# palonso/MAEST

Measured on AMD Instinct MI355X. Metric: clips/sec (10s@16kHz, 96-mel) MAEST-10s fwd+bwd, higher is better.
Workload: dtype bf16; 1 GPU; maest_10s_random_weights_pretrain training step (BASELINE configs[2]): mixup + fwd + BCE + bwd + AdamW; arch=passt_s_swa_p16_128_ap476 (DeiT-B distilled, 85.9M params), random init, per_gpu_batch=256, global_batch=256, s_patchout_t=30, classes=400, hip_graph_forward=False, parallelism=dp1

## Files before the change

maest_amd/csrc/embed.hip:

```cpp
#include "common.h"

namespace maest {

constexpr int PE_D = 768;
constexpr int PE_K = 16;
constexpr int PE_S = 10;

__device__ __forceinline__ uint32_t stripe_bits(const int32_t* __restrict__ t_stripes, int n_t,
                                                const int32_t* __restrict__ f_stripes, int n_f, int b, int frow,
                                                int tcol) {
    for (int k = 0; k < n_f; ++k) {
        int st = f_stripes[((int64_t)b * n_f + k) * 2];
        const int w = f_stripes[((int64_t)b * n_f + k) * 2 + 1];
        st = st < 0 ? 0 : st;
        if (frow >= st && frow < st + w) return 0xffffu;
    }
    uint32_t bits = 0;
    for (int k = 0; k < n_t; ++k) {
        int st = t_stripes[((int64_t)b * n_t + k) * 2];
        const int w = t_stripes[((int64_t)b * n_t + k) * 2 + 1];
        st = st < 0 ? 0 : st;
        int lo = st - tcol, hi = st + w - tcol;
        lo = lo < 0 ? 0 : lo;
        hi = hi > 16 ? 16 : hi;
// ... 77 lines not shown
    const int c = threadIdx.x * 4;
    const int b0 = blockIdx.y * TA_BCHUNK;
    const int b1 = b0 + TA_BCHUNK < B ? b0 + TA_BCHUNK : B;
    if (n < 2) {
        const float* tok = n == 0 ? cls_token : dist_token;
        float4 o;
        o.x = tok[c] + new_pos[n * PE_D + c];
        o.y = tok[c + 1] + new_pos[n * PE_D + c + 1];
        o.z = tok[c + 2] + new_pos[n * PE_D + c + 2];
        o.w = tok[c + 3] + new_pos[n * PE_D + c + 3];
        for (int b = b0; b < b1; ++b) *reinterpret_cast<float4*>(x0 + ((int64_t)b * Ntok + n) * PE_D + c) = o;
        return;
    }
    const int j = n - 2;
    const int f = tok_ft[2 * j];
    const int tcol = toffset + tok_ft[2 * j + 1];
    float tp[4], fp[4];
#pragma unroll
    for (int e = 0; e < 4; ++e) {
        tp[e] = time_pos[(int64_t)(c + e) * Tt + tcol];
        fp[e] = freq_pos[(int64_t)(c + e) * Fg + f];
    }
    for (int b = b0; b < b1; ++b) {
        const float4 p = *reinterpret_cast<const float4*>(patches + ((int64_t)b * P + j) * PE_D + c);
        float4 o;
        o.x = (p.x + tp[0]) + fp[0];
        o.y = (p.y + tp[1]) + fp[1];
        o.z = (p.z + tp[2]) + fp[2];
        o.w = (p.w + tp[3]) + fp[3];
        *reinterpret_cast<float4*>(x0 + ((int64_t)b * Ntok + n) * PE_D + c) = o;
    }
}

constexpr int TAB_SLICES = 2;
template <bool TABLES>
__global__ __launch_bounds__(192) void token_assemble_bwd_kernel(const float* __restrict__ dx0, int B, int Fg, int P,
                                                                 int Tt, int toffset,
                                                                 const int32_t* __restrict__ tok_ft,
                                                                 void* __restrict__ dpatches, int dtype,
                                                                 float* __restrict__ d_cls, float* __restrict__ d_dist,
                                                                 float* __restrict__ d_new_pos,
                                                                 float* __restrict__ d_freq_pos,
                                                                 float* __restrict__ d_time_pos) {
    const int Ntok = 2 + P;
    const int n = TABLES ? blockIdx.x : blockIdx.x + 2;
    const int c = threadIdx.x * 4;
    const int per = (B + (int)gridDim.y - 1) / (int)gridDim.y;
    const int b0 = blockIdx.y * per;
    const int b1 = b0 + per < B ? b0 + per : B;
    float s[4] = {0.0f, 0.0f, 0.0f, 0.0f};
    const bool store = n >= 2 && dpatches != nullptr;
    auto one = [&](int b, const float4& g) {
        s[0] += g.x; s[1] += g.y; s[2] += g.z; s[3] += g.w;
        if (store) {
            const int64_t o = ((int64_t)b * P + (n - 2)) * PE_D + c;
            if (dtype == MAEST_BF16) {
                chunk8 v;
                v[0] = pack_bf2(g.x, g.y); v[1] = pack_bf2(g.z, g.w);
                *reinterpret_cast<chunk8*>(reinterpret_cast<bf16_t*>(dpatches) + o) = v;
            } else {
                *reinterpret_cast<float4*>(reinterpret_cast<float*>(dpatches) + o) = g;
            }
        }
    };
    const int64_t bstride = (int64_t)Ntok * PE_D;
    const float* src = dx0 + (int64_t)n * PE_D + c;
    int b = b0;
    for (; b + 4 <= b1; b += 4) {
        float4 g[4];
#pragma unroll
        for (int u = 0; u < 4; ++u) g[u] = *reinterpret_cast<const float4*>(src + (b + u) * bstride);
#pragma unroll
        for (int u = 0; u < 4; ++u) one(b + u, g[u]);
    }
    for (; b < b1; ++b) one(b, *reinterpret_cast<const float4*>(src + b * bstride));
    if (!TABLES || b0 >= b1) return;
    if (n == 0) {
#pragma unroll
        for (int e = 0; e < 4; ++e) { unsafeAtomicAdd(d_cls + c + e, s[e]); unsafeAtomicAdd(d_new_pos + c + e, s[e]); }
    } else if (n == 1) {
#pragma unroll
        for (int e = 0; e < 4; ++e) { unsafeAtomicAdd(d_dist + c + e, s[e]); unsafeAtomicAdd(d_new_pos + PE_D + c + e, s[e]); }
    } else {
        const int j = n - 2;
        const int f = tok_ft[2 * j];
        const int tcol = toffset + tok_ft[2 * j + 1];
#pragma unroll
        for (int e = 0; e < 4; ++e) {
            unsafeAtomicAdd(d_freq_pos + (int64_t)(c + e) * Fg + f, s[e]);
            unsafeAtomicAdd(d_time_pos + (int64_t)(c + e) * Tt + tcol, s[e]);
        }
    }
}

__global__ __launch_bounds__(64) void token_tables_ordered_kernel(const float* __restrict__ dx0, int B, int Fg, int P, int Tt, int toffset,
                                                                  const int32_t* __restrict__ tok_ft, float* __restrict__ d_cls,
                                                                  float* __restrict__ d_dist, float* __restrict__ d_new_pos,
                                                                  float* __restrict__ d_freq_pos, float* __restrict__ d_time_pos) {
    const int Ntok = 2 + P;
    const int d = blockIdx.x;
    const int c = blockIdx.y * 256 + threadIdx.x * 4;
    const int64_t bstride = (int64_t)Ntok * PE_D;
    float s[4] = {0.0f, 0.0f, 0.0f, 0.0f};
    auto token = [&](int n) {
        const float* src = dx0 + (int64_t)n * PE_D + c;
        int b = 0;
        for (; b + 16 <= B; b += 16) {
            float4 g[16];
#pragma unroll
// ... 235 lines not shown
    int32_t* mlist = lam ? moff + B + 1 : nullptr;
    hipLaunchKernelGGL(col2im_prep_kernel, dim3(1), dim3(256), 0, (hipStream_t)stream, tok_ft, P, Fp, Tp, perm, B, lut, moff,
                       mlist);
    const dim3 grid((unsigned)(((int64_t)F * T + 255) / 256), (unsigned)B);
#define MAEST_COL2IM(GT, XT)                                                                                               \
    hipLaunchKernelGGL((col2im_kernel<GT, XT>), grid, dim3(256), 0, (hipStream_t)stream, (const GT*)dcols, B, F, T,       \
                       stride_f, stride_t, Fp, Tp, P, lam, lut, moff, mlist, t_stripes, n_t, f_stripes, n_f, (XT*)dx)
    if (dtype == MAEST_BF16 && dx_dtype == MAEST_F16) MAEST_COL2IM(bf16_t, _Float16);
    else if (dtype == MAEST_BF16) MAEST_COL2IM(bf16_t, float);
    else if (dx_dtype == MAEST_F16) MAEST_COL2IM(float, _Float16);
    else MAEST_COL2IM(float, float);
#undef MAEST_COL2IM
    return check_launch("maest_patch_im2col_bwd");
}

extern "C" int maest_token_assemble(const float* patches, const float* cls_token, const float* dist_token,
                                    const float* new_pos, const float* freq_pos, const float* time_pos, int Fg, int Tt,
                                    int toffset, const int32_t* tok_ft, int B, int P, float* x0, void* stream) {
    MAEST_REQUIRE(patches && cls_token && dist_token && new_pos && freq_pos && time_pos && x0 && tok_ft,
                  "maest_token_assemble: null pointer");
    MAEST_REQUIRE(B > 0 && P > 0 && Fg > 0 && Tt > 0 && toffset >= 0, "maest_token_assemble: bad shape");
    hipLaunchKernelGGL(token_assemble_kernel, dim3(2 + P, (B + TA_BCHUNK - 1) / TA_BCHUNK), dim3(PE_D / 4), 0,
                       (hipStream_t)stream, patches, cls_token, dist_token, new_pos, freq_pos, time_pos, Tt, toffset,
                       tok_ft, B, Fg, P, x0);
    return check_launch("maest_token_assemble");
}

extern "C" int maest_token_assemble_bwd(const float* dx0, int B, int P, int Fg, int Tt, int toffset,
                                        const int32_t* tok_ft, void* dpatches, int dtype, float* d_cls, float* d_dist,
                                        float* d_new_pos, float* d_freq_pos, float* d_time_pos, void* stream) {
    MAEST_REQUIRE(dx0 && d_cls && d_dist && d_new_pos && d_freq_pos && d_time_pos && tok_ft,
                  "maest_token_assemble_bwd: null pointer");
    MAEST_REQUIRE(B > 0 && P > 0 && Fg > 0 && Tt > 0, "maest_token_assemble_bwd: bad shape");
    static_assert(PE_D == 192 * 4, "token_assemble_bwd_kernel: one thread per four channels");
    if (option(MAEST_OPT_DETERMINISTIC) != 0) {
        if (dpatches != nullptr)
            hipLaunchKernelGGL(token_assemble_bwd_kernel<false>, dim3(P, TAB_SLICES), dim3(192), 0, (hipStream_t)stream, dx0, B, Fg, P, Tt,
                               toffset, tok_ft, dpatches, dtype, d_cls, d_dist, d_new_pos, d_freq_pos, d_time_pos);
        static_assert(PE_D == 3 * 256, "token_tables_ordered_kernel: three channel groups of 64 lanes x 4");
        hipLaunchKernelGGL(token_tables_ordered_kernel, dim3(2 + Fg + Tt, 3), dim3(64), 0, (hipStream_t)stream, dx0, B, Fg, P, Tt, toffset,
                           tok_ft, d_cls, d_dist, d_new_pos, d_freq_pos, d_time_pos);
        return check_launch("maest_token_assemble_bwd(ordered)");
    }
    hipLaunchKernelGGL(token_assemble_bwd_kernel<true>, dim3(2 + P, TAB_SLICES), dim3(192), 0, (hipStream_t)stream,
                       dx0, B, Fg, P, Tt, toffset, tok_ft, dpatches, dtype, d_cls, d_dist, d_new_pos, d_freq_pos,
                       d_time_pos);
    return check_launch("maest_token_assemble_bwd");
}

extern "C" int maest_spec_mask(float* x, int B, int F, int T, const int32_t* t_stripes, int n_t,
                               const int32_t* f_stripes, int n_f, void* stream) {
    MAEST_REQUIRE(x, "maest_spec_mask: null pointer");
    MAEST_REQUIRE(n_t >= 0 && n_f >= 0 && (n_t == 0 || t_stripes) && (n_f == 0 || f_stripes),
                  "maest_spec_mask: bad stripe lists");
    if (n_t + n_f == 0) return MAEST_OK;
    hipLaunchKernelGGL(spec_mask_kernel, dim3(B, n_t + n_f), dim3(256), 0, (hipStream_t)stream, x, F, T, t_stripes,
                       n_t, f_stripes, n_f);
    return check_launch("maest_spec_mask");
}

extern "C" int maest_melfile_assemble(const uint16_t* frames, const int64_t* row_start, const int32_t* frames_read,
                                      int B, int n_bands, int T, int normalize, float norm_mean, float norm_div,
                                      float* out, void* stream) {
    MAEST_REQUIRE(frames && row_start && frames_read && out, "maest_melfile_assemble: null pointer");
    MAEST_REQUIRE(B > 0 && T > 0 && n_bands > 0 && n_bands <= 96, "maest_melfile_assemble: bad shape B=%d T=%d bands=%d",
                  B, T, n_bands);
    hipLaunchKernelGGL(melfile_assemble_kernel, dim3((T + 63) / 64, B), dim3(256), 64 * 97 * 4, (hipStream_t)stream, frames,
                       row_start, frames_read, n_bands, T, normalize, norm_mean, norm_div, out);
    return check_launch("maest_melfile_assemble");
}
```

maest_amd/csrc/gemm.hip:

```cpp
#include "common.h"
#include "gemm256_epi.h"

namespace maest {

constexpr int GEMM_BM = 128;
constexpr int GEMM_BN = 128;
constexpr int GEMM_ROWB = 128;
constexpr int GEMM_PITCH = 144;
constexpr int GEMM_TILE_BYTES = GEMM_BM * GEMM_PITCH;
constexpr int GEMM_SMEM_BYTES = 4 * GEMM_TILE_BYTES;

struct GemmParams {
    const char* A;
    const char* B;
    void* C;
    const float* bias;
    const void* aux_in;
    void* aux_out;
    float* colsum;
    int64_t lda, ldb, ldc, ld_aux;
    int M, N, K;
    int out_dtype;
    int epi;
    int vec_ok;
// ... 20 lines not shown
        for (int g = 0; g < 4; ++g) {
            const int nl = wn * 64 + jn * 32 + 8 * g + 4 * h;
            float b4[4] = {0.0f, 0.0f, 0.0f, 0.0f};
            if (bias != nullptr && n0 + nl < N) {
                const float4 t = *reinterpret_cast<const float4*>(bias + n0 + nl);
                b4[0] = t.x; b4[1] = t.y; b4[2] = t.z; b4[3] = t.w;
            }
#pragma unroll
            for (int im = 0; im < 2; ++im) {
                const int ml = wm * 64 + im * 32 + (lane & 31);
                float v[4];
#pragma unroll
                for (int e = 0; e < 4; ++e) {
                    v[e] = acc[jn][im][4 * g + e] + b4[e];
                    if (GMODE != 0) {
                        float gv, dv;
                        gelu_pair<EXACT>(v[e], gv, dv);
                        v[e] = GMODE == 1 ? gv : dv;
                    }
                }
                char* dst = smem + ml * E::PITCH + nl * OSZ;
                if (OSZ == 4) {
                    *reinterpret_cast<float4*>(dst) = make_float4(v[0], v[1], v[2], v[3]);
                } else {
                    chunk8 o;
                    o[0] = pack_bf2(v[0], v[1]);
                    o[1] = pack_bf2(v[2], v[3]);
                    *reinterpret_cast<chunk8*>(dst) = o;
                }
            }
        }
}

template <int OSZ, int MODE>
__device__ __forceinline__ void epi_drain(const char* smem, void* dst, int64_t ld, const void* aux, int64_t ld_aux,
                                          int m0, int n0, int M, int N, int tid) {
    using E = EpiCfg<OSZ>;
#pragma unroll 4
    for (int c = tid; c < 128 * E::CPR; c += 256) {
        const int row = c / E::CPR, cc = c - row * E::CPR;
        const int gm = m0 + row, gn = n0 + cc * E::EPC;
        if (gm >= M || gn >= N) continue;
        chunk16 v = *reinterpret_cast<const chunk16*>(smem + row * E::PITCH + cc * 16);
        if (MODE == 1) {
            const float4 r = *reinterpret_cast<const float4*>(reinterpret_cast<const float*>(aux) + (int64_t)gm * ld_aux + gn);
            v[0] = f2u(u2f(v[0]) + r.x); v[1] = f2u(u2f(v[1]) + r.y);
            v[2] = f2u(u2f(v[2]) + r.z); v[3] = f2u(u2f(v[3]) + r.w);
        } else if (MODE == 2) {
            if (OSZ == 4) {
                const float4 r = *reinterpret_cast<const float4*>(reinterpret_cast<const float*>(aux) + (int64_t)gm * ld_aux + gn);
                v[0] = f2u(u2f(v[0]) * r.x); v[1] = f2u(u2f(v[1]) * r.y);
                v[2] = f2u(u2f(v[2]) * r.z); v[3] = f2u(u2f(v[3]) * r.w);
            } else {
                const chunk16 r = *reinterpret_cast<const chunk16*>(reinterpret_cast<const bf16_t*>(aux) + (int64_t)gm * ld_aux + gn);
#pragma unroll
                for (int e = 0; e < 4; ++e) {
                    const uint32_t vw = v[e], rw = r[e];
                    const float lo = bf2f((bf16_t)(vw & 0xffffu)) * bf2f((bf16_t)(rw & 0xffffu));
                    const float hi = bf2f((bf16_t)(vw >> 16)) * bf2f((bf16_t)(rw >> 16));
                    v[e] = pack_bf2(lo, hi);
                }
            }
        }
        __builtin_nontemporal_store(v, reinterpret_cast<chunk16*>(reinterpret_cast<char*>(dst) + ((int64_t)gm * ld + gn) * OSZ));
    }
}

__device__ __forceinline__ void epi_drain_mul16(const char* smem, void* dst, int64_t ld, const void* aux, int64_t ld_aux,
                                                int m0, int n0, int M, int N, int tid) {
    using E = EpiCfg<2>;
#pragma unroll 4
    for (int c = tid; c < 128 * E::CPR; c += 256) {
        const int row = c / E::CPR, cc = c - row * E::CPR;
        const int gm = m0 + row, gn = n0 + cc * E::EPC;
        if (gm >= M || gn >= N) continue;
        const chunk16 r = *reinterpret_cast<const chunk16*>(reinterpret_cast<const bf16_t*>(aux) + (int64_t)gm * ld_aux + gn);
        const chunk16 v = mul16_chunk(smem + row * EpiCfg<4>::PITCH + cc * 32, r);
        __builtin_nontemporal_store(v, reinterpret_cast<chunk16*>(reinterpret_cast<char*>(dst) + ((int64_t)gm * ld + gn) * 2));
    }
}

template <int OSZ, bool EXACT>
__device__ __forceinline__ void epi_vector(char* smem, const f32x16_t (&acc)[2][2], const GemmParams& p, int m0, int n0,
                                           int wm, int wn, int lane, int tid) {
    switch (p.epi) {
        case MAEST_EPI_GELU:
            if (p.aux_out != nullptr) {
                epi_stage<OSZ, 2, EXACT>(smem, acc, p.bias, n0, p.N, wm, wn, lane);
                __syncthreads();
                epi_drain<OSZ, 0>(smem, p.aux_out, p.ld_aux, nullptr, 0, m0, n0, p.M, p.N, tid);
                __syncthreads();
            }
            epi_stage<OSZ, 1, EXACT>(smem, acc, p.bias, n0, p.N, wm, wn, lane);
            __syncthreads();
            epi_drain<OSZ, 0>(smem, p.C, p.ldc, nullptr, 0, m0, n0, p.M, p.N, tid);
            break;
        case MAEST_EPI_RESIDUAL:
            epi_stage<OSZ, 0, EXACT>(smem, acc, p.bias, n0, p.N, wm, wn, lane);
            __syncthreads();
            epi_drain<OSZ, 1>(smem, p.C, p.ldc, p.aux_in, p.ld_aux, m0, n0, p.M, p.N, tid);
            break;
        case MAEST_EPI_MUL:
            if constexpr (OSZ == 2) {
                epi_stage<4, 0, EXACT>(smem, acc, p.bias, n0, p.N, wm, wn, lane);
                __syncthreads();
                epi_drain_mul16(smem, p.C, p.ldc, p.aux_in, p.ld_aux, m0, n0, p.M, p.N, tid);
            } else {
                epi_stage<OSZ, 0, EXACT>(smem, acc, p.bias, n0, p.N, wm, wn, lane);
                __syncthreads();
                epi_drain<OSZ, 2>(smem, p.C, p.ldc, p.aux_in, p.ld_aux, m0, n0, p.M, p.N, tid);
            }
            break;
        default:
            epi_stage<OSZ, 0, EXACT>(smem, acc, p.bias, n0, p.N, wm, wn, lane);
            __syncthreads();
            epi_drain<OSZ, 0>(smem, p.C, p.ldc, nullptr, 0, m0, n0, p.M, p.N, tid);
            break;
    }
}

template <bool EXACT>
__device__ __forceinline__ void epi_scalar(const f32x16_t (&acc)[2][2], const GemmParams& p, int m0, int n0, int wm,
                                           int wn, int lane, bool add_bias) {
#pragma unroll
    for (int im = 0; im < 2; ++im) {
        const int row = m0 + wm * 64 + im * 32 + (lane & 31);
        if (row >= p.M) continue;
#pragma unroll
        for (int jn = 0; jn < 2; ++jn)
#pragma unroll
            for (int r = 0; r < 16; ++r) {
                const int col = n0 + wn * 64 + jn * 32 + frag_row(r, lane);
                if (col >= p.N) continue;
                float v = acc[jn][im][r] + ((p.bias != nullptr && add_bias) ? p.bias[col] : 0.0f);
                const int64_t ci = (int64_t)row * p.ldc + col;
                const int64_t xi = (int64_t)row * p.ld_aux + col;
                switch (p.epi) {
                    case MAEST_EPI_GELU: {
                        float gv, dv;
                        gelu_pair<EXACT>(v, gv, dv);
                        if (p.aux_out != nullptr) {
                            if (p.out_dtype == MAEST_BF16) reinterpret_cast<bf16_t*>(p.aux_out)[xi] = f2bf(dv);
                            else reinterpret_cast<float*>(p.aux_out)[xi] = dv;
                        }
                        v = gv;
                        break;
                    }
                    case MAEST_EPI_RESIDUAL:
                        v += reinterpret_cast<const float*>(p.aux_in)[xi];
// ... 102 lines not shown
        for (int ks = 0; ks < 4; ++ks) {
            const int coff = (2 * ks + h) * 16;
            chunk16 fa[2], fb[2];
#pragma unroll
            for (int i = 0; i < 2; ++i) {
                fa[i] = *reinterpret_cast<const chunk16*>(la + a_rd + i * 32 * GEMM_PITCH + coff);
                fb[i] = *reinterpret_cast<const chunk16*>(lb + b_rd + i * 32 * GEMM_PITCH + coff);
            }
#pragma unroll
            for (int jn = 0; jn < 2; ++jn)
#pragma unroll
                for (int im = 0; im < 2; ++im) mma_chunk<T>(acc[jn][im], fb[jn], fa[im]);
        }
        if (more) {
            char* da = smem + (cur ^ 1) * 2 * GEMM_TILE_BYTES;
#pragma unroll
            for (int i = 0; i < 4; ++i) {
                *reinterpret_cast<chunk16*>(da + st_off + i * 32 * GEMM_PITCH) = ra[i];
                *reinterpret_cast<chunk16*>(da + GEMM_TILE_BYTES + st_off + i * 32 * GEMM_PITCH) = rb[i];
            }
        }
        __syncthreads();
    }

    if (p.vec_ok && p.epi != MAEST_EPI_ATOMIC) {
        constexpr bool EXACT = sizeof(T) == 4;
        if (p.out_dtype == MAEST_BF16) epi_vector<2, EXACT>(smem, acc, p, m0, n0, wm, wn, lane, tid);
        else epi_vector<4, EXACT>(smem, acc, p, m0, n0, wm, wn, lane, tid);
    } else {
        epi_scalar<sizeof(T) == 4>(acc, p, m0, n0, wm, wn, lane, blockIdx.y == 0);
    }
}

template <typename T>
struct TnCfg {
    static constexpr int ELT = (int)sizeof(T);
    static constexpr int KS = 128 / ELT;
    static constexpr int ROWB = 128 * ELT;
    static constexpr int PITCH = ELT == 2 ? 320 : 528;
    static constexpr int CPR = ROWB / 16;
    static constexpr int RPP = 256 / CPR;
    static constexpr int EPC = 16 / ELT;
    static constexpr int TILE = KS * PITCH;
    static constexpr int SMEM = 4 * TILE;
};

typedef short v4i16_t __attribute__((ext_vector_type(4)));

template <typename T>
__device__ __forceinline__ chunk16 load_frag_tn(const char* tile, int ks, int iblk, int lane);
template <>
__device__ __forceinline__ chunk16 load_frag_tn<bf16_t>(const char* tile, int ks, int iblk, int lane) {
    using C = TnCfg<bf16_t>;
    const int h = lane >> 5, g16 = (lane >> 4) & 1, q = lane & 15;
    const char* p = tile + (ks * 16 + 8 * h + (q >> 2)) * C::PITCH + (iblk + 16 * g16 + 4 * (q & 3)) * 2;
    const v4i16_t lo = __builtin_amdgcn_ds_read_tr16_b64_v4i16((__attribute__((address_space(3))) v4i16_t*)(p));
    const v4i16_t hi = __builtin_amdgcn_ds_read_tr16_b64_v4i16((__attribute__((address_space(3))) v4i16_t*)(p + 4 * C::PITCH));
    const chunk8 l2 = __builtin_bit_cast(chunk8, lo), h2 = __builtin_bit_cast(chunk8, hi);
    chunk16 c;
    c[0] = l2[0]; c[1] = l2[1]; c[2] = h2[0]; c[3] = h2[1];
    return c;
}
template <>
__device__ __forceinline__ chunk16 load_frag_tn<float>(const char* tile, int ks, int iblk, int lane) {
    using C = TnCfg<float>;
    const int h = lane >> 5;
// ... 207 lines not shown
int64_t gemm_tn256_workspace_bytes(int dtype, int M, int N, int K, int split_k);

template <typename T>
__global__ __launch_bounds__(256) void rowdot_kernel(const T* __restrict__ c_mat, int64_t ldc, const T* __restrict__ other,
                                                     int64_t ld_other, float* __restrict__ rowdot, int M, int groups, int ntok) {
    const int64_t gid = (int64_t)blockIdx.x * 256 + threadIdx.x;
    const int64_t total = (int64_t)M * groups;
    int64_t item = gid >> 2;
    const int quarter = (int)(gid & 3);
    const bool valid = item < total;
    if (!valid) item = total - 1;
    const int64_t row = item / groups;
    const int g = (int)(item - row * groups);
    const T* pc = c_mat + row * ldc + g * 64 + quarter * 16;
    const T* po = other + row * ld_other + g * 64 + quarter * 16;
    float acc = 0.0f;
#pragma unroll
    for (int i = 0; i < 16; ++i) acc += elem_traits<T>::to_f32(pc[i]) * elem_traits<T>::to_f32(po[i]);
    acc += __shfl_xor(acc, 1, 64);
    acc += __shfl_xor(acc, 2, 64);
    if (valid && quarter == 0) {
        const int64_t it = row / ntok, q = row - it * ntok;
        rowdot[(it * groups + g) * ntok + q] = acc;
    }
}

template <typename T>
static int launch_gemm_nt(GemmParams& p, int split_k, hipStream_t stream) {
    static DeviceOnce once;
    ensure_dynamic_lds(once, &gemm_nt_kernel<T>, GEMM_SMEM_BYTES);
    dim3 grid(p.tiles_m * p.tiles_n, split_k, 1);
    hipLaunchKernelGGL(gemm_nt_kernel<T>, grid, dim3(256), GEMM_SMEM_BYTES, stream, p);
    return check_launch("maest_gemm_nt");
}

template <typename T>
static int launch_gemm_tn(GemmParams& p, int split_k, hipStream_t stream) {
    static DeviceOnce once;
    ensure_dynamic_lds(once, &gemm_tn_kernel<T>, TnCfg<T>::SMEM);
    dim3 grid(p.tiles_m * p.tiles_n, split_k, 1);
    hipLaunchKernelGGL(gemm_tn_kernel<T>, grid, dim3(256), TnCfg<T>::SMEM, stream, p);
    return check_launch("maest_gemm_tn");
}
template <typename T>
static int launch_gemm_tn_ws(GemmParams& p, int split_k, hipStream_t stream) {
    static DeviceOnce once;
    ensure_dynamic_lds(once, &gemm_tn_kernel<T, true>, TnCfg<T>::SMEM);
    dim3 grid(p.tiles_m * p.tiles_n, split_k, 1);
    hipLaunchKernelGGL((gemm_tn_kernel<T, true>), grid, dim3(256), TnCfg<T>::SMEM, stream, p);
    const int rc = check_launch("maest_gemm_tn(ordered)");
    if (rc != MAEST_OK) return rc;
    const int64_t n = (int64_t)p.M * p.N + (p.colsum != nullptr ? p.M : 0);
    hipLaunchKernelGGL(tn_small_reduce_kernel, dim3((unsigned)((n + 255) / 256)), dim3(256), 0, stream, (const float*)p.ws,
                       reinterpret_cast<float*>(p.C), p.ldc, p.M, p.N, (int64_t)p.tiles_m * 128, (int64_t)p.tiles_n * 128, split_k, p.colsum);
    return check_launch("maest_gemm_tn(ordered, reduce)");
}

static void tn_small_plan(int dtype, int M, int N, int K, int split_k, int* splits, int* per_split) {
    if (split_k == 0) {
        const int t = ((M + 127) / 128) * ((N + 127) / 128);
        split_k = 1024 / t > 0 ? 1024 / t : 1;
    }
    const int ks = 128 / (dtype == MAEST_BF16 ? 2 : 4);
    const int total = (K + ks - 1) / ks;
    if (split_k > total) split_k = total;
    *per_split = (total + split_k - 1) / split_k;
// ... 30 lines not shown
    MAEST_REQUIRE(epi >= MAEST_EPI_NONE && epi <= MAEST_EPI_ATOMIC, "maest_gemm_nt: bad epilogue %d", epi);
    MAEST_REQUIRE(split_k >= 1, "maest_gemm_nt: split_k must be >= 1");
    MAEST_REQUIRE(split_k == 1 || epi == MAEST_EPI_ATOMIC, "maest_gemm_nt: split_k > 1 needs MAEST_EPI_ATOMIC");
    MAEST_REQUIRE(epi != MAEST_EPI_ATOMIC || out_dtype == MAEST_F32, "maest_gemm_nt: atomic epilogue accumulates fp32");
    MAEST_REQUIRE(split_k == 1 || option(MAEST_OPT_DETERMINISTIC) == 0,
                  "maest_gemm_nt: split_k > 1 combines its partials with atomics in an order that varies from run to run: not available under "
                  "MAEST_OPT_DETERMINISTIC (use split_k = 1)");
    MAEST_REQUIRE(epi != MAEST_EPI_RESIDUAL || (aux_in && out_dtype == MAEST_F32), "maest_gemm_nt: residual epilogue needs fp32 aux_in and fp32 out");
    MAEST_REQUIRE(epi != MAEST_EPI_MUL || aux_in, "maest_gemm_nt: mul epilogue needs aux_in");
    GemmParams p;
    p.A = (const char*)A; p.B = (const char*)B; p.C = C;
    p.bias = bias; p.aux_in = aux_in; p.aux_out = aux_out; p.colsum = nullptr; p.ws = nullptr;
    p.lda = lda; p.ldb = ldb; p.ldc = ldc; p.ld_aux = ld_aux;
    p.M = M; p.N = N; p.K = K;
    p.out_dtype = out_dtype; p.epi = epi;
    const int osz = out_dtype == MAEST_F32 ? 4 : 2;
    const int epc = 16 / osz;
    bool vec = (N % epc == 0) && (N % 4 == 0) && (ldc % epc == 0) && ((uintptr_t)C % 16 == 0);
    if (bias) vec = vec && ((uintptr_t)bias % 16 == 0);
    if (aux_out) vec = vec && (ld_aux % epc == 0) && ((uintptr_t)aux_out % 16 == 0);
    if (aux_in) {
        const int aepc = (epi == MAEST_EPI_RESIDUAL) ? 4 : epc;
        vec = vec && (ld_aux % aepc == 0) && ((uintptr_t)aux_in % 16 == 0);
    }
    p.vec_ok = vec ? 1 : 0;
    if (vec && split_k == 1) {
        const int rc = gemm_nt256_try(A, lda, B, ldb, x3 ? MAEST_F32X3 : in_dtype, C, ldc, out_dtype, M, N, K, bias, epi,
                                      aux_in, aux_out, ld_aux, (hipStream_t)stream);
        if (rc >= 0) return rc;
    }
    if (split_out) p.vec_ok = 0;
    p.tiles_m = (M + GEMM_BM - 1) / GEMM_BM;
    p.tiles_n = (N + GEMM_BN - 1) / GEMM_BN;
    const int total = K / ks;
    if (split_k > total) split_k = total;
    p.k_slices_per_split = (total + split_k - 1) / split_k;
    split_k = (total + p.k_slices_per_split - 1) / p.k_slices_per_split;
    return in_dtype == MAEST_BF16 ? launch_gemm_nt<bf16_t>(p, split_k, (hipStream_t)stream)
                                  : launch_gemm_nt<float>(p, split_k, (hipStream_t)stream);
}

extern "C" int maest_gemm_nt_rowdot(const void* A, int64_t lda, const void* B, int64_t ldb, int in_dtype, void* C,
                                    int64_t ldc, int out_dtype, int M, int N, int K, const float* bias, const void* other,
                                    int64_t ld_other, float* rowdot, int rows_per_item, void* stream) {
    MAEST_REQUIRE(A && B && C && other && rowdot, "maest_gemm_nt_rowdot: null pointer");
    MAEST_REQUIRE(M > 0 && N > 0 && K > 0 && (N % 64) == 0, "maest_gemm_nt_rowdot: bad shape M=%d N=%d K=%d (N %% 64 == 0)", M, N, K);
    MAEST_REQUIRE(rows_per_item > 0 && (M % rows_per_item) == 0, "maest_gemm_nt_rowdot: M=%d is not a multiple of rows_per_item=%d",
                  M, rows_per_item);
    MAEST_REQUIRE(out_dtype == MAEST_F32 || out_dtype == MAEST_BF16, "maest_gemm_nt_rowdot: bad out_dtype %d", out_dtype);
    const int osz = out_dtype == MAEST_BF16 ? 2 : 4, epc = 16 / osz;
    MAEST_REQUIRE((ld_other % epc) == 0 && ((uintptr_t)other % 16) == 0 && (ldc % epc) == 0 && ((uintptr_t)C % 16) == 0,
                  "maest_gemm_nt_rowdot: C / other rows must be 16-byte aligned");
    const bool x3 = in_dtype == MAEST_F32X3;
    const int in_plain = x3 ? MAEST_F32 : in_dtype;
    MAEST_REQUIRE(in_plain == MAEST_F32 || in_plain == MAEST_BF16, "maest_gemm_nt_rowdot: bad in_dtype %d", in_dtype);
    const int elt = in_plain == MAEST_BF16 ? 2 : 4;
    if (K % (GEMM_ROWB / elt) == 0 && (lda * elt) % 16 == 0 && (ldb * elt) % 16 == 0 && ((uintptr_t)A % 16) == 0 &&
        ((uintptr_t)B % 16) == 0 && (bias == nullptr || ((uintptr_t)bias % 16) == 0)) {
        const int rc = gemm_nt256_try(A, lda, B, ldb, in_dtype, C, ldc, out_dtype, M, N, K, bias, MAEST_EPI_ROWDOT, other,
                                      nullptr, ld_other, (hipStream_t)stream, rowdot, rows_per_item);
        if (rc >= 0) return rc;
    }
    const int rc = maest_gemm_nt(A, lda, B, ldb, in_dtype, C, ldc, out_dtype, M, N, K, bias, MAEST_EPI_NONE, nullptr, nullptr,
                                 0, 1, stream);
    if (rc != MAEST_OK) return rc;
    const int groups = N / 64;
// ... 92 lines not shown
```

maest_amd/csrc/gemm256.hip:

```cpp
#include <cstdlib>
#include <type_traits>

#include "common.h"
#include "gemm256_epi.h"

namespace maest {

constexpr int G2_ROWB = 64;
constexpr int G2_TILE = 256 * G2_ROWB;
constexpr int G2_STAGES = 4;
constexpr int G2_SMEM = G2_STAGES * 2 * G2_TILE;
#define MAEST_WAIT_VMCNT(N) __builtin_amdgcn_s_waitcnt(((N) & 15) | (((N) >> 4) << 14) | 0x0F70)


template <int OSZ>
struct Epi256 {
    static constexpr int PITCH = 256 * OSZ + 16;
    static constexpr int ROWS = OSZ == 2 ? 128 : 64;
    static constexpr int MT = ROWS / 32;
    static constexpr int PASSES = 256 / ROWS;
    static constexpr int CPR = 256 * OSZ / 16;
    static constexpr int EPC = 16 / OSZ;
};

// ... 840 lines not shown
        for (int q = 0; q < 4; ++q) s[q] += __builtin_nontemporal_load(reinterpret_cast<const f32x4_t*>(src + q * 256));
        src += step;
    }
    float* cp = C + ((int64_t)tile_i * 256 + wm * 128 + a * 32) * ldc + tile_j * 256 + (OW ? wn * 128 : wn * 64) + b * 32 + (lane & 31);
    float old[16];
#pragma unroll
    for (int r = 0; r < 16; ++r) old[r] = cp[(int64_t)frag_row(r, lane) * ldc];
#pragma unroll
    for (int r = 0; r < 16; ++r) cp[(int64_t)frag_row(r, lane) * ldc] = old[r] + s[r >> 2][r & 3];
}

__global__ __launch_bounds__(256) void tn256_colsum_reduce_kernel(const float* __restrict__ cs_ws, float* __restrict__ colsum, int M, int n) {
    const int m = blockIdx.x * 256 + threadIdx.x;
    if (m >= M) return;
    const float* src = cs_ws + m;
    float s = 0.0f;
    int i = 0;
    for (; i + 4 <= n; i += 4) {
        const float v0 = src[0], v1 = src[M], v2 = src[2 * (int64_t)M], v3 = src[3 * (int64_t)M];
        s += v0; s += v1; s += v2; s += v3;
        src += 4 * (int64_t)M;
    }
    for (; i < n; ++i) {
        s += src[0];
        src += M;
    }
    colsum[m] = colsum[m] + s;
}

static bool tn256_plan(int dtype, int M, int N, int K, int split_k, int* splits, int* per_split) {
    if (dtype == MAEST_F32X3) dtype = MAEST_F32;
    const int ks = dtype == MAEST_BF16 ? Tn256<bf16_t>::KS : Tn256<float>::KS;
    if ((M % 256) != 0 || (N % 256) != 0 || (K % ks) != 0 || K < 8 * ks) return false;
    if ((int64_t)M * N < (int64_t)8 * 65536 && option(MAEST_OPT_GEMM_VARIANT) != 4)
        return false;
    const int total = K / ks;
    const int tiles = (M / 256) * (N / 256);
    if (split_k <= 0) split_k = tiles >= 256 ? 1 : 256 / tiles;
    if (split_k > total / 4) split_k = total / 4 > 0 ? total / 4 : 1;
    *per_split = (total + split_k - 1) / split_k;
    *splits = (total + *per_split - 1) / *per_split;
    return true;
}

int64_t gemm_tn256_workspace_bytes(int dtype, int M, int N, int K, int split_k) {
    int splits = 1, per = 0;
    const bool ordered = option(MAEST_OPT_DETERMINISTIC) != 0;
    if ((option(MAEST_OPT_TN_REDUCE) == 0 && !ordered) || !tn256_plan(dtype, M, N, K, split_k, &splits, &per) || splits < 2) return 0;
    const int64_t c_bytes = (int64_t)splits * (M / 256) * (N / 256) * 65536 * (int64_t)sizeof(float);
    return ordered ? c_bytes + (int64_t)splits * (N / 256) * M * (int64_t)sizeof(float) : c_bytes;
}

static int launch_tn256_reduce(const GemmTn256Params& p, int split_k, bool ow, hipStream_t stream) {
    const int ntiles = p.tiles_m * p.tiles_n;
    if (ow)
        hipLaunchKernelGGL(tn256_reduce_kernel<true>, dim3(ntiles * 64), dim3(64), 0, stream, (const float*)p.ws, p.C, p.ldc, ntiles,
                           p.tiles_n, split_k);
    else
        hipLaunchKernelGGL(tn256_reduce_kernel<false>, dim3(ntiles * 64), dim3(64), 0, stream, (const float*)p.ws, p.C, p.ldc, ntiles,
                           p.tiles_n, split_k);
    int rc = check_launch("maest_gemm_tn(256, reduce)");
    if (rc != MAEST_OK || p.cs_ws == nullptr || p.colsum == nullptr) return rc;
    hipLaunchKernelGGL(tn256_colsum_reduce_kernel, dim3((p.M + 255) / 256), dim3(256), 0, stream, (const float*)p.cs_ws, p.colsum, p.M,
                       split_k * p.tiles_n);
    return check_launch("maest_gemm_tn(256, colsum reduce)");
}

template <typename T, bool X3 = false>
static int launch_tn256(GemmTn256Params& p, int split_k, hipStream_t stream) {
    static DeviceOnce once;
    ensure_dynamic_lds(once, &gemm_tn256_kernel<T, X3>, G2_SMEM);
// ... 45 lines not shown
```

Measured before the change: 5728 clips/s.

## Add split-K small NT GEMM, enable TN256 for small long-K, rework token bwd reduce

Adds a 64x64-tile NT GEMM kernel for small-M bf16 problems. Its four waves each take a slice of K and combine their partials through LDS before a shared epilogue. The epilogue helpers are templated on tile size so this kernel can reuse them. TN256 planning now also accepts small-output, long-K bf16 weight-gradient GEMMs, using 128/tiles splits. The token-assemble backward kernel now splits channels across blocks and batch across waves with an LDS reduction, issuing fewer atomics. Each path adds new launch heuristics that could pick a slower kernel for some shapes.

```diff
diff --git a/maest_amd/csrc/embed.hip b/maest_amd/csrc/embed.hip
--- a/maest_amd/csrc/embed.hip
+++ b/maest_amd/csrc/embed.hip
@@ -133,9 +133,9 @@
     }
 }
 
-constexpr int TAB_SLICES = 2;
+constexpr int TAB_WAVES = 4;
 template <bool TABLES>
-__global__ __launch_bounds__(192) void token_assemble_bwd_kernel(const float* __restrict__ dx0, int B, int Fg, int P,
+__global__ __launch_bounds__(64 * TAB_WAVES) void token_assemble_bwd_kernel(const float* __restrict__ dx0, int B, int Fg, int P,
                                                                  int Tt, int toffset,
                                                                  const int32_t* __restrict__ tok_ft,
                                                                  void* __restrict__ dpatches, int dtype,
@@ -143,11 +143,14 @@
                                                                  float* __restrict__ d_new_pos,
                                                                  float* __restrict__ d_freq_pos,
                                                                  float* __restrict__ d_time_pos) {
+    extern __shared__ __attribute__((aligned(16))) char smem[];
+    float4* part = reinterpret_cast<float4*>(smem);
     const int Ntok = 2 + P;
     const int n = TABLES ? blockIdx.x : blockIdx.x + 2;
-    const int c = threadIdx.x * 4;
-    const int per = (B + (int)gridDim.y - 1) / (int)gridDim.y;
-    const int b0 = blockIdx.y * per;
+    const int lane = threadIdx.x & 63, w = threadIdx.x >> 6;
+    const int c = blockIdx.y * 256 + lane * 4;
+    const int per = (B + TAB_WAVES - 1) / TAB_WAVES;
+    const int b0 = w * per;
     const int b1 = b0 + per < B ? b0 + per : B;
     float s[4] = {0.0f, 0.0f, 0.0f, 0.0f};
     const bool store = n >= 2 && dpatches != nullptr;
@@ -167,15 +170,23 @@
     const int64_t bstride = (int64_t)Ntok * PE_D;
     const float* src = dx0 + (int64_t)n * PE_D + c;
     int b = b0;
-    for (; b + 4 <= b1; b += 4) {
-        float4 g[4];
-#pragma unroll
-        for (int u = 0; u < 4; ++u) g[u] = *reinterpret_cast<const float4*>(src + (b + u) * bstride);
-#pragma unroll
-        for (int u = 0; u < 4; ++u) one(b + u, g[u]);
+    for (; b + 8 <= b1; b += 8) {
+        float4 g[8];
+#pragma unroll
+        for (int u = 0; u < 8; ++u) g[u] = *reinterpret_cast<const float4*>(src + (b + u) * bstride);
+#pragma unroll
+        for (int u = 0; u < 8; ++u) one(b + u, g[u]);
     }
     for (; b < b1; ++b) one(b, *reinterpret_cast<const float4*>(src + b * bstride));
-    if (!TABLES || b0 >= b1) return;
+    if (!TABLES) return;
+    part[w * 64 + lane] = make_float4(s[0], s[1], s[2], s[3]);
+    __syncthreads();
+    if (w != 0) return;
+#pragma unroll
+    for (int v = 1; v < TAB_WAVES; ++v) {
+        const float4 q = part[v * 64 + lane];
+        s[0] += q.x; s[1] += q.y; s[2] += q.z; s[3] += q.w;
+    }
     if (n == 0) {
 #pragma unroll
         for (int e = 0; e < 4; ++e) { unsafeAtomicAdd(d_cls + c + e, s[e]); unsafeAtomicAdd(d_new_pos + c + e, s[e]); }
@@ -477,17 +488,16 @@
     MAEST_REQUIRE(dx0 && d_cls && d_dist && d_new_pos && d_freq_pos && d_time_pos && tok_ft,
                   "maest_token_assemble_bwd: null pointer");
     MAEST_REQUIRE(B > 0 && P > 0 && Fg > 0 && Tt > 0, "maest_token_assemble_bwd: bad shape");
-    static_assert(PE_D == 192 * 4, "token_assemble_bwd_kernel: one thread per four channels");
+    static_assert(PE_D == 3 * 256, "token_assemble_bwd_kernel: three channel groups of 64 lanes x 4");
     if (option(MAEST_OPT_DETERMINISTIC) != 0) {
         if (dpatches != nullptr)
-            hipLaunchKernelGGL(token_assemble_bwd_kernel<false>, dim3(P, TAB_SLICES), dim3(192), 0, (hipStream_t)stream, dx0, B, Fg, P, Tt,
+            hipLaunchKernelGGL(token_assemble_bwd_kernel<false>, dim3(P, 3), dim3(64 * TAB_WAVES), 0, (hipStream_t)stream, dx0, B, Fg, P, Tt,
                                toffset, tok_ft, dpatches, dtype, d_cls, d_dist, d_new_pos, d_freq_pos, d_time_pos);
-        static_assert(PE_D == 3 * 256, "token_tables_ordered_kernel: three channel groups of 64 lanes x 4");
         hipLaunchKernelGGL(token_tables_ordered_kernel, dim3(2 + Fg + Tt, 3), dim3(64), 0, (hipStream_t)stream, dx0, B, Fg, P, Tt, toffset,
                            tok_ft, d_cls, d_dist, d_new_pos, d_freq_pos, d_time_pos);
         return check_launch("maest_token_assemble_bwd(ordered)");
     }
-    hipLaunchKernelGGL(token_assemble_bwd_kernel<true>, dim3(2 + P, TAB_SLICES), dim3(192), 0, (hipStream_t)stream,
+    hipLaunchKernelGGL(token_assemble_bwd_kernel<true>, dim3(2 + P, 3), dim3(64 * TAB_WAVES), TAB_WAVES * 64 * 16, (hipStream_t)stream,
                        dx0, B, Fg, P, Tt, toffset, tok_ft, dpatches, dtype, d_cls, d_dist, d_new_pos, d_freq_pos,
                        d_time_pos);
     return check_launch("maest_token_assemble_bwd");
diff --git a/maest_amd/csrc/gemm.hip b/maest_amd/csrc/gemm.hip
--- a/maest_amd/csrc/gemm.hip
+++ b/maest_amd/csrc/gemm.hip
@@ -76,13 +76,14 @@
         }
 }
 
-template <int OSZ, int MODE>
+template <int OSZ, int MODE, int TILE = 128>
 __device__ __forceinline__ void epi_drain(const char* smem, void* dst, int64_t ld, const void* aux, int64_t ld_aux,
                                           int m0, int n0, int M, int N, int tid) {
     using E = EpiCfg<OSZ>;
+    constexpr int CPR = TILE * OSZ / 16;
 #pragma unroll 4
-    for (int c = tid; c < 128 * E::CPR; c += 256) {
-        const int row = c / E::CPR, cc = c - row * E::CPR;
+    for (int c = tid; c < TILE * CPR; c += 256) {
+        const int row = c / CPR, cc = c - row * CPR;
         const int gm = m0 + row, gn = n0 + cc * E::EPC;
         if (gm >= M || gn >= N) continue;
         chunk16 v = *reinterpret_cast<const chunk16*>(smem + row * E::PITCH + cc * 16);
@@ -110,12 +111,14 @@
     }
 }
 
+template <int TILE = 128>
 __device__ __forceinline__ void epi_drain_mul16(const char* smem, void* dst, int64_t ld, const void* aux, int64_t ld_aux,
                                                 int m0, int n0, int M, int N, int tid) {
     using E = EpiCfg<2>;
+    constexpr int CPR = TILE * 2 / 16;
 #pragma unroll 4
-    for (int c = tid; c < 128 * E::CPR; c += 256) {
-        const int row = c / E::CPR, cc = c - row * E::CPR;
+    for (int c = tid; c < TILE * CPR; c += 256) {
+        const int row = c / CPR, cc = c - row * CPR;
         const int gm = m0 + row, gn = n0 + cc * E::EPC;
         if (gm >= M || gn >= N) continue;
         const chunk16 r = *reinterpret_cast<const chunk16*>(reinterpret_cast<const bf16_t*>(aux) + (int64_t)gm * ld_aux + gn);
@@ -124,41 +127,42 @@
     }
 }
 
-template <int OSZ, bool EXACT>
+template <int OSZ, bool EXACT, int TILE = 128>
 __device__ __forceinline__ void epi_vector(char* smem, const f32x16_t (&acc)[2][2], const GemmParams& p, int m0, int n0,
                                            int wm, int wn, int lane, int tid) {
+    const bool stager = TILE == 128 || tid < 64;
     switch (p.epi) {
         case MAEST_EPI_GELU:
             if (p.aux_out != nullptr) {
-                epi_stage<OSZ, 2, EXACT>(smem, acc, p.bias, n0, p.N, wm, wn, lane);
+                if (stager) epi_stage<OSZ, 2, EXACT>(smem, acc, p.bias, n0, p.N, wm, wn, lane);
                 __syncthreads();
-                epi_drain<OSZ, 0>(smem, p.aux_out, p.ld_aux, nullptr, 0, m0, n0, p.M, p.N, tid);
+                epi_drain<OSZ, 0, TILE>(smem, p.aux_out, p.ld_aux, nullptr, 0, m0, n0, p.M, p.N, tid);
                 __syncthreads();
             }
-            epi_stage<OSZ, 1, EXACT>(smem, acc, p.bias, n0, p.N, wm, wn, lane);
+            if (stager) epi_stage<OSZ, 1, EXACT>(smem, acc, p.bias, n0, p.N, wm, wn, lane);
             __syncthreads();
-            epi_drain<OSZ, 0>(smem, p.C, p.ldc, nullptr, 0, m0, n0, p.M, p.N, tid);
+            epi_drain<OSZ, 0, TILE>(smem, p.C, p.ldc, nullptr, 0, m0, n0, p.M, p.N, tid);
             break;
         case MAEST_EPI_RESIDUAL:
-            epi_stage<OSZ, 0, EXACT>(smem, acc, p.bias, n0, p.N, wm, wn, lane);
+            if (stager) epi_stage<OSZ, 0, EXACT>(smem, acc, p.bias, n0, p.N, wm, wn, lane);
             __syncthreads();
-            epi_drain<OSZ, 1>(smem, p.C, p.ldc, p.aux_in, p.ld_aux, m0, n0, p.M, p.N, tid);
+            epi_drain<OSZ, 1, TILE>(smem, p.C, p.ldc, p.aux_in, p.ld_aux, m0, n0, p.M, p.N, tid);
             break;
         case MAEST_EPI_MUL:
             if constexpr (OSZ == 2) {
-                epi_stage<4, 0, EXACT>(smem, acc, p.bias, n0, p.N, wm, wn, lane);
+                if (stager) epi_stage<4, 0, EXACT>(smem, acc, p.bias, n0, p.N, wm, wn, lane);
                 __syncthreads();
-                epi_drain_mul16(smem, p.C, p.ldc, p.aux_in, p.ld_aux, m0, n0, p.M, p.N, tid);
+                epi_drain_mul16<TILE>(smem, p.C, p.ldc, p.aux_in, p.ld_aux, m0, n0, p.M, p.N, tid);
             } else {
-                epi_stage<OSZ, 0, EXACT>(smem, acc, p.bias, n0, p.N, wm, wn, lane);
+                if (stager) epi_stage<OSZ, 0, EXACT>(smem, acc, p.bias, n0, p.N, wm, wn, lane);
                 __syncthreads();
-                epi_drain<OSZ, 2>(smem, p.C, p.ldc, p.aux_in, p.ld_aux, m0, n0, p.M, p.N, tid);
+                epi_drain<OSZ, 2, TILE>(smem, p.C, p.ldc, p.aux_in, p.ld_aux, m0, n0, p.M, p.N, tid);
             }
             break;
         default:
-            epi_stage<OSZ, 0, EXACT>(smem, acc, p.bias, n0, p.N, wm, wn, lane);
+            if (stager) epi_stage<OSZ, 0, EXACT>(smem, acc, p.bias, n0, p.N, wm, wn, lane);
             __syncthreads();
-            epi_drain<OSZ, 0>(smem, p.C, p.ldc, nullptr, 0, m0, n0, p.M, p.N, tid);
+            epi_drain<OSZ, 0, TILE>(smem, p.C, p.ldc, nullptr, 0, m0, n0, p.M, p.N, tid);
             break;
     }
 }
@@ -327,6 +331,113 @@
     }
 }
 
+constexpr int NTS_MAX_M = 512;
+constexpr int NTS_MAX_TILES128 = 64;
+constexpr int NTS_TILE = 64;
+constexpr int NTS_STAGE = 64;
+constexpr int NTS_DEPTH = 4;
+constexpr int NTS_SMEM_BYTES = 3 * NTS_TILE * NTS_TILE * 4;
+static_assert(NTS_TILE * EpiCfg<4>::PITCH <= NTS_SMEM_BYTES, "the staged tile must fit the partials' bytes");
+
+template <typename T>
+__global__ __launch_bounds__(256) void gemm_nt_small_kernel(GemmParams p) {
+    extern __shared__ __attribute__((aligned(16))) char smem[];
+    const int tid = threadIdx.x;
+    const int lane = tid & 63;
+    const int wave = tid >> 6;
+    const int h = lane >> 5;
+    constexpr int ELT = (int)sizeof(T);
+
+    const int wg = xcd_remap(blockIdx.x, p.tiles_m * p.tiles_n);
+    const int tile_n = wg / p.tiles_m;
+    const int tile_m = wg - tile_n * p.tiles_m;
+    const int m0 = tile_m * NTS_TILE, n0 = tile_n * NTS_TILE;
+
+    const int nst = (int)((int64_t)p.K * ELT / NTS_STAGE);
+    const int per = (nst + 3) / 4;
+    const int s0 = wave * per;
+    const int s1 = s0 + per < nst ? s0 + per : nst;
+    const int n = s1 > s0 ? s1 - s0 : 0;
+
+    const char* a_src[2];
+    const char* b_src[2];
+#pragma unroll
+    for (int i = 0; i < 2; ++i) {
+        int ra = m0 + 32 * i + (lane & 31);
+        if (ra > p.M - 1) ra = p.M - 1;
+        int rb = n0 + 32 * i + (lane & 31);
+        if (rb > p.N - 1) rb = p.N - 1;
+        a_src[i] = p.A + (int64_t)ra * p.lda * ELT + (int64_t)s0 * NTS_STAGE + h * 16;
+        b_src[i] = p.B + (int64_t)rb * p.ldb * ELT + (int64_t)s0 * NTS_STAGE + h * 16;
+    }
+
+    f32x16_t acc[2][2];
+#pragma unroll
+    for (int i = 0; i < 2; ++i)
+#pragma unroll
+        for (int j = 0; j < 2; ++j)
+#pragma unroll
+            for (int r = 0; r < 16; ++r) acc[i][j][r] = 0.0f;
+
+    chunk16 fa[NTS_DEPTH][2][2], fb[NTS_DEPTH][2][2];
+#define NTS_LOAD(u, s)                                                                                            \
+    _Pragma("unroll") for (int ks = 0; ks < 2; ++ks) _Pragma("unroll") for (int i = 0; i < 2; ++i) {               \
+        fa[u][ks][i] = *reinterpret_cast<const chunk16*>(a_src[i] + (int64_t)(s) * NTS_STAGE + ks * 32);          \
+        fb[u][ks][i] = *reinterpret_cast<const chunk16*>(b_src[i] + (int64_t)(s) * NTS_STAGE + ks * 32);          \
+    }
+#pragma unroll
+    for (int u = 0; u < NTS_DEPTH; ++u)
+        if (u < n) { NTS_LOAD(u, u) }
+    for (int s = 0; s < n; s += NTS_DEPTH) {
+#pragma unroll
+        for (int u = 0; u < NTS_DEPTH; ++u) {
+            if (s + u < n) {
+#pragma unroll
+                for (int ks = 0; ks < 2; ++ks)
+#pragma unroll
+                    for (int jn = 0; jn < 2; ++jn)
+#pragma unroll
+                        for (int im = 0; im < 2; ++im) mma_chunk<T>(acc[jn][im], fb[u][ks][jn], fa[u][ks][im]);
+                if (s + u + NTS_DEPTH < n) { NTS_LOAD(u, s + u + NTS_DEPTH) }
+            }
+        }
+    }
+#undef NTS_LOAD
+
+    float4* part = reinterpret_cast<float4*>(smem);
+    if (wave != 0) {
+#pragma unroll
+        for (int b = 0; b < 4; ++b)
+#pragma unroll
+            for (int q = 0; q < 4; ++q)
+                part[((wave - 1) * 16 + b * 4 + q) * 64 + lane] =
+                    make_float4(acc[b >> 1][b & 1][4 * q], acc[b >> 1][b & 1][4 * q + 1], acc[b >> 1][b & 1][4 * q + 2], acc[b >> 1][b & 1][4 * q + 3]);
+    }
+    __syncthreads();
+    if (wave == 0) {
+#pragma unroll
+        for (int v = 0; v < 3; ++v)
+#pragma unroll
+            for (int b = 0; b < 4; ++b)
+#pragma unroll
+                for (int q = 0; q < 4; ++q) {
+                    const float4 t = part[(v * 16 + b * 4 + q) * 64 + lane];
+                    acc[b >> 1][b & 1][4 * q] += t.x;
+                    acc[b >> 1][b & 1][4 * q + 1] += t.y;
+                    acc[b >> 1][b & 1][4 * q + 2] += t.z;
+                    acc[b >> 1][b & 1][4 * q + 3] += t.w;
+                }
+    }
+    __syncthreads();
+    constexpr bool EXACT = sizeof(T) == 4;
+    if (p.vec_ok) {
+        if (p.out_dtype == MAEST_BF16) epi_vector<2, EXACT, NTS_TILE>(smem, acc, p, m0, n0, 0, 0, lane, tid);
+        else epi_vector<4, EXACT, NTS_TILE>(smem, acc, p, m0, n0, 0, 0, lane, tid);
+    } else if (wave == 0) {
+        epi_scalar<EXACT>(acc, p, m0, n0, 0, 0, lane, true);
+    }
+}
+
 template <typename T>
 struct TnCfg {
     static constexpr int ELT = (int)sizeof(T);
@@ -600,6 +711,16 @@
     dim3 grid(p.tiles_m * p.tiles_n, split_k, 1);
     hipLaunchKernelGGL(gemm_nt_kernel<T>, grid, dim3(256), GEMM_SMEM_BYTES, stream, p);
     return check_launch("maest_gemm_nt");
+}
+
+template <typename T>
+static int launch_gemm_nt_small(GemmParams& p, hipStream_t stream) {
+    static DeviceOnce once;
+    ensure_dynamic_lds(once, &gemm_nt_small_kernel<T>, NTS_SMEM_BYTES);
+    p.tiles_m = (p.M + NTS_TILE - 1) / NTS_TILE;
+    p.tiles_n = (p.N + NTS_TILE - 1) / NTS_TILE;
+    hipLaunchKernelGGL(gemm_nt_small_kernel<T>, dim3(p.tiles_m * p.tiles_n), dim3(256), NTS_SMEM_BYTES, stream, p);
+    return check_launch("maest_gemm_nt(small)");
 }
 
 template <typename T>
@@ -696,6 +817,8 @@
     if (split_out) p.vec_ok = 0;
     p.tiles_m = (M + GEMM_BM - 1) / GEMM_BM;
     p.tiles_n = (N + GEMM_BN - 1) / GEMM_BN;
+    if (in_dtype == MAEST_BF16 && M <= NTS_MAX_M && p.tiles_m * p.tiles_n < NTS_MAX_TILES128 && split_k == 1 && epi != MAEST_EPI_ATOMIC)
+        return launch_gemm_nt_small<bf16_t>(p, (hipStream_t)stream);
     const int total = K / ks;
     if (split_k > total) split_k = total;
     p.k_slices_per_split = (total + split_k - 1) / split_k;
diff --git a/maest_amd/csrc/gemm256.hip b/maest_amd/csrc/gemm256.hip
--- a/maest_amd/csrc/gemm256.hip
+++ b/maest_amd/csrc/gemm256.hip
@@ -896,11 +896,12 @@
     if (dtype == MAEST_F32X3) dtype = MAEST_F32;
     const int ks = dtype == MAEST_BF16 ? Tn256<bf16_t>::KS : Tn256<float>::KS;
     if ((M % 256) != 0 || (N % 256) != 0 || (K % ks) != 0 || K < 8 * ks) return false;
-    if ((int64_t)M * N < (int64_t)8 * 65536 && option(MAEST_OPT_GEMM_VARIANT) != 4)
-        return false;
     const int total = K / ks;
     const int tiles = (M / 256) * (N / 256);
-    if (split_k <= 0) split_k = tiles >= 256 ? 1 : 256 / tiles;
+    const bool few = (int64_t)M * N < (int64_t)8 * 65536;
+    const bool few_long = few && dtype == MAEST_BF16 && total >= 256 && option(MAEST_OPT_DETERMINISTIC) == 0 && option(MAEST_OPT_TN_REDUCE) == 0;
+    if (few && !few_long && option(MAEST_OPT_GEMM_VARIANT) != 4) return false;
+    if (split_k <= 0) split_k = tiles >= 256 ? 1 : (few_long ? 128 : 256) / tiles;
     if (split_k > total / 4) split_k = total / 4 > 0 ? total / 4 : 1;
     *per_split = (total + split_k - 1) / split_k;
     *splits = (total + *per_split - 1) / *per_split;
```

After: 5746 clips/s, median of 6. Within noise of the previous version (+0.3%).
